# AITRICS/Medical_Tri_Modal_Pilot

Hardware: AMD Instinct MI355X
Metric: tri-modal training samples/s (fwd+bwd+AdamW step, per-GPU batch 64) (higher is better)
Workload: dtype bf16; 1 GPU; BASELINE configs[1]: vslt_img_txt tri_mbt_vsltcls, 6 layers, d_model 256, batch 64/GPU, TIE-len 1000 (N_v=1005), 224x224 CXR, 128-tok text, dropout 0.1, mbt-only-vslt 1, imgtxt-time 1; global_batch=64, parallelism=dp1

## Files before the change

### include/mtmp.h

```cpp
#ifndef MTMP_H
#define MTMP_H
#include <stdint.h>
#ifdef __cplusplus
extern "C" {
#endif

#define MTMP_F32 0
#define MTMP_BF16 1

int mtmp_abi_version(void);
const char* mtmp_last_error(void);

int mtmp_attn_fwd(int dtype, const void* q, const void* k, const void* v, void* o, const void* res, void* o_res,
                  float* lse, const int32_t* kv_len, const float* key_norms, int B, int N, int H, int ld_qkv, int ld_o,
                  float scale, void* stream);
int mtmp_attn_fwd_grouped(int dtype, int n, const void* const* q, const void* const* k, const void* const* v, void* const* o,
                          const void* const* res, void* const* o_res, float* const* lse, const int32_t* const* kv_len,
                          const int32_t* const* row_start, const float* const* key_norms, const int* N, const int* ld_qkv,
                          const int* ld_o, int B, int H, float scale, void* stream);
int mtmp_attn_bwd_grouped(int dtype, int n, const void* const* q, const void* const* k, const void* const* v,
                          const void* const* o, const void* const* d_o, const float* const* lse, const int32_t* const* kv_len,
                          const int32_t* const* row_start, void* const* dq, void* const* dk, void* const* dv,
                          float* const* delta_ws, const int* N, const int* ld_qkv, const int* ld_o, const int* ld_do,
                          const int* ld_dqkv, int B, int H, float scale, void* stream);
int mtmp_attn_cls_fwd(int dtype, const void* q, const void* k, const void* v, int ld_qkv, const void* res, int ld_res, void* o_cls,
                      void* r1_cls, float* lse, const int32_t* kv_len, const int32_t* row_start, int B, int N, int H, int cls_tok,
                      float scale, void* stream);
int mtmp_attn_cls_bwd(int dtype, const void* q, const void* k, const void* v, int ld_qkv, const void* o_cls, const void* d_o,
                      const float* lse, const int32_t* kv_len, const int32_t* row_start, void* dq, void* dk, void* dv, int ld_dqkv,
                      int B, int N, int H, int cls_tok, float scale, void* stream);
long long mtmp_key_norms_floats(long long rows, int H);
int mtmp_key_norms(int dtype, const void* k, float* out, long long rows, int H, int ld, void* stream);

int mtmp_attn_bwd(int dtype, const void* q, const void* k, const void* v, const void* o, const void* d_o,
                  const float* lse, const int32_t* kv_len, void* dq, void* dk, void* dv, float* delta_ws, int B,
                  int N, int H, int ld_qkv, int ld_o, int ld_do, int ld_dqkv, float scale, void* stream);

int mtmp_ln_gemm(int dtype, const void* x, const float* gamma, const float* beta, const void* w, const float* bias,
                 void* y, void* xn, float* stats, int M, int N, int ldx, int ldy, float eps, int relu, float drop_p,
                 unsigned seed, const unsigned* seed_dev, void* stream);

int mtmp_ln_gemm_qkv(int dtype, const void* x, const float* gamma, const float* beta, const void* w, const float* bias,
                     void* y, void* xn, float* stats, float* key_norms, int M, int ldx, float eps, void* stream);

int mtmp_gemm_nt(int dtype, const void* a, const void* w, const float* bias, const void* res, void* y, int M, int N,
                 int K, int lda, int ldy, int ldr, int act, float drop_p, unsigned seed, const unsigned* seed_dev,
                 const void* gate, float gate_scale, const float* row_scale, int rows_per_scale, void* stream);

long long mtmp_sign_bits_bytes(int M, int N);
int mtmp_ln_gemm_signs(int dtype, const void* x, const float* gamma, const float* beta, const void* w, const float* bias,
                       void* y, void* xn, float* stats, int M, int N, int ldx, int ldy, float eps, float drop_p,
                       unsigned seed, const unsigned* seed_dev, void* signs, void* stream);
int mtmp_gemm_nt_signs(int dtype, const void* a, const void* w, void* y, int M, int N, int lda, int ldy,
                       const void* signs, float gate_scale, void* stream);
int mtmp_gemm_nt_signs_drop(int dtype, const void* a, const void* w, void* y, int M, int N, int lda, int ldy,
                            const void* signs, float gate_scale, float drop_p, unsigned seed, const unsigned* seed_dev,
                            void* a_out, void* stream);

long long mtmp_gemm_tn_ws_floats(int M, int N, int K);
int mtmp_gemm_tn(int dtype, const void* dy, const void* x, float* dw, float* db, float* ws, int M, int N, int K,
                 int ldy, int ldx, void* stream);
int mtmp_gemm_tn_live(int dtype, const void* dy, const void* x, float* dw, float* db, float* ws, int M, int N, int K,
                      int ldy, int ldx, const int32_t* rows_live, void* stream);

int mtmp_dropout_bwd(int dtype, const void* g_in, void* g_out, long long n, unsigned seed, const unsigned* seed_dev,
                     float p, void* stream);

int mtmp_ln_bwd_ws_floats(int M);
int mtmp_ln_bwd(int dtype, const void* z, int ldz, const float* stats, const float* gamma, const void* dy,
                const void* d_res, int ldr, void* dz, float* dgamma_dbeta, float* ws, int M, float eps, void* stream);

int mtmp_gemm_lnbwd_ws_floats(int M);
int mtmp_gemm_lnbwd(int dtype, const void* dy, const void* wt, const void* z, int ldz, const float* stats,
                    const float* gamma, const void* d_res, int ldr, void* dz, float* dgamma_dbeta, float* ws, int M,
                    int K, int ldy, float eps, void* stream);

int mtmp_tie_embed_fwd(int dtype, const float* events, const float* params, const float* ftab, void* out, int n,
                       void* stream);
int mtmp_tie_bwd_ws_floats(int n);
int mtmp_tie_embed_bwd(int dtype, const float* events, const float* params, const void* d_out, float* grads,
                       float* ws, int n, void* stream);

int mtmp_time_embed_fwd(int dtype, const float* events, const float* params, const float* ftab, void* out, int n,
// ... 163 lines not shown
```

### medical_tri_modal_pilot_amd/_lib.py

```python
import ctypes
import os
from ctypes import c_char_p, c_float, c_int, c_longlong, c_uint, c_void_p

_HERE = os.path.dirname(os.path.abspath(__file__))
LIB_PATH = os.environ.get("MTMP_LIB", os.path.join(_HERE, "libmtmp_hip.so"))

F32, BF16 = 0, 1

SIGNATURES = {
    "mtmp_abi_version": (c_int, []),
    "mtmp_last_error": (c_char_p, []),
    "mtmp_attn_fwd": (c_int, [c_int] + [c_void_p] * 9 + [c_int] * 5 + [c_float, c_void_p]),
    "mtmp_attn_cls_fwd": (c_int, [c_int] + [c_void_p] * 3 + [c_int, c_void_p, c_int] + [c_void_p] * 5 + [c_int] * 4 + [c_float, c_void_p]),
    "mtmp_attn_cls_bwd": (c_int, [c_int] + [c_void_p] * 3 + [c_int] + [c_void_p] * 8 + [c_int] * 5 + [c_float, c_void_p]),
    "mtmp_attn_fwd_grouped": (c_int, [c_int, c_int] + [c_void_p] * 13 + [c_int, c_int, c_float, c_void_p]),
    "mtmp_attn_bwd_grouped": (c_int, [c_int, c_int] + [c_void_p] * 17 + [c_int, c_int, c_float, c_void_p]),
    "mtmp_key_norms_floats": (c_longlong, [c_longlong, c_int]),
    "mtmp_key_norms": (c_int, [c_int, c_void_p, c_void_p, c_longlong, c_int, c_int, c_void_p]),
    "mtmp_attn_bwd": (c_int, [c_int] + [c_void_p] * 11 + [c_int] * 7 + [c_float, c_void_p]),
    "mtmp_ln_gemm": (c_int, [c_int] + [c_void_p] * 8 + [c_int] * 4 + [c_float, c_int, c_float, c_uint, c_void_p, c_void_p]),
    "mtmp_ln_gemm_qkv": (c_int, [c_int] + [c_void_p] * 9 + [c_int, c_int, c_float, c_void_p]),
    "mtmp_gemm_nt": (c_int, [c_int] + [c_void_p] * 5 + [c_int] * 7 + [c_float, c_uint, c_void_p, c_void_p, c_float, c_void_p, c_int,
                             c_void_p]),
    "mtmp_gemm_nt_live": (c_int, [c_int] + [c_void_p] * 5 + [c_int] * 7 + [c_float, c_uint, c_void_p, c_void_p, c_float, c_void_p, c_int,
                             c_void_p, c_void_p]),
    "mtmp_sign_bits_bytes": (c_longlong, [c_int, c_int]),
    "mtmp_ln_gemm_signs": (c_int, [c_int] + [c_void_p] * 8 + [c_int] * 4 + [c_float, c_float, c_uint, c_void_p, c_void_p, c_void_p]),
    "mtmp_gemm_nt_signs": (c_int, [c_int] + [c_void_p] * 3 + [c_int] * 4 + [c_void_p, c_float, c_void_p]),
    "mtmp_gemm_nt_signs_drop": (c_int, [c_int] + [c_void_p] * 3 + [c_int] * 4 + [c_void_p, c_float, c_float, c_uint, c_void_p,
                                                                                   c_void_p, c_void_p]),
    "mtmp_ln_gemm_qkv_grouped": (c_int, [c_int, c_int] + [c_void_p] * 11 + [c_float, c_void_p, c_void_p]),
    "mtmp_ln_gemm_signs_grouped": (c_int, [c_int, c_int] + [c_void_p] * 10 + [c_int, c_void_p, c_float, c_float, c_void_p, c_void_p,
                                                                                   c_void_p, c_void_p]),
    "mtmp_gemm_nt_grouped": (c_int, [c_int, c_int] + [c_void_p] * 6 + [c_int, c_int] + [c_void_p] * 3 + [c_int, c_float, c_void_p,
                                                                                                       c_void_p, c_void_p, c_void_p]),
    "mtmp_gemm_nt_signs_drop_grouped": (c_int, [c_int, c_int] + [c_void_p] * 4 + [c_int, c_void_p, c_void_p, c_float, c_float,
                                                                                  c_void_p, c_void_p, c_void_p, c_void_p, c_void_p]),
    "mtmp_gemm_lnbwd_grouped": (c_int, [c_int, c_int] + [c_void_p] * 11 + [c_int, c_void_p, c_float, c_void_p, c_void_p]),
    "mtmp_gemm_tn_group_plan": (c_int, [c_int, c_void_p, c_int, c_int, c_void_p]),
    "mtmp_gemm_tn_grouped": (c_int, [c_int, c_int] + [c_void_p] * 4 + [c_int, c_int] + [c_void_p] * 4 + [c_void_p]),
    "mtmp_gemm_tn_slab_rows": (c_int, [c_int] * 4),
    "mtmp_gemm_lnbwd_slab_rows": (c_int, [c_int]),
    "mtmp_reduce_batch": (c_int, [c_void_p] * 6 + [c_int, c_void_p]),
    "mtmp_reduce_scatter": (c_int, [c_void_p] * 5 + [c_int, c_void_p]),
    "mtmp_stream_input_slab_rows": (c_int, [c_int]),
    "mtmp_stream_input_bwd_partials": (c_int, [c_int] + [c_void_p] * 7 + [c_int] * 3 + [c_float, c_uint, c_void_p, c_void_p, c_void_p, c_void_p]),
    "mtmp_stream_input_bwd_grouped": (c_int, [c_int, c_int] + [c_void_p] * 18),
    "mtmp_stream_input_fwd_add": (c_int, [c_int] + [c_void_p] * 8 + [c_int] * 3 + [c_float, c_float, c_uint, c_void_p, c_void_p, c_void_p, c_void_p, c_int, c_void_p]),
    "mtmp_token_sums": (c_int, [c_int, c_int] + [c_void_p] * 5),
    "mtmp_tie_bwd_slab_rows": (c_int, [c_int]),
    "mtmp_tie_time_embed_bwd_partials": (c_int, [c_int, c_void_p, c_int, c_void_p, c_int, c_int] + [c_void_p] * 6),
    "mtmp_publish_scalar": (c_int, [c_void_p, c_void_p, c_void_p]),
    "mtmp_copy_batch": (c_int, [c_void_p] * 4 + [c_int, c_void_p]),
    "mtmp_stream_lengths": (c_int, [c_void_p] * 4 + [c_int] * 3 + [c_void_p]),
    "mtmp_row_starts": (c_int, [c_void_p, c_void_p, c_int, c_int, c_void_p]),
    "mtmp_image_slots": (c_int, [c_void_p, c_int, c_void_p, c_int, c_int, c_void_p]),
    "mtmp_transpose_batch": (c_int, [c_int, c_void_p, c_void_p, c_void_p, c_void_p, c_int, c_void_p]),
    "mtmp_layernorm_rows": (c_int, [c_int] + [c_void_p] * 4 + [c_longlong, c_int, c_float, c_int, c_int, c_int, c_void_p]),
    "mtmp_layernorm_rows_live": (c_int, [c_int] + [c_void_p] * 4 + [c_longlong, c_int, c_float, c_int, c_int, c_int, c_void_p, c_void_p]),
    "mtmp_swin_window_attn": (c_int, [c_int] + [c_void_p] * 3 + [c_int] * 6 + [c_float, c_void_p]),
    "mtmp_swin_window_attn_live": (c_int, [c_int] + [c_void_p] * 3 + [c_int] * 6 + [c_float, c_void_p, c_void_p]),
    "mtmp_layernorm_rows_bwd_slab_rows": (c_int, [c_longlong, c_int]),
    "mtmp_layernorm_rows_bwd": (c_int, [c_int] + [c_void_p] * 5 + [c_longlong, c_int, c_float, c_void_p]),
    "mtmp_gelu_fwd": (c_int, [c_int, c_void_p, c_void_p, c_longlong, c_void_p]),
    "mtmp_gelu_bwd": (c_int, [c_int, c_void_p, c_void_p, c_void_p, c_longlong, c_void_p]),
    "mtmp_swin_window_attn_bwd": (c_int, [c_int] + [c_void_p] * 5 + [c_int] * 6 + [c_float, c_void_p]),
    "mtmp_swin_window_attn_pad": (c_int, [c_int] + [c_void_p] * 4 + [c_int] * 6 + [c_float, c_void_p, c_void_p]),
# ... 67 lines not shown
```

### medical_tri_modal_pilot_amd/ops.py

```python
import contextlib
import ctypes
from typing import Optional

import torch

from . import _lib, tuning
from ._lib import BF16, F32, call

LN_EPS = 1e-6
N_HEAD, D_MODEL, D_HEAD = 4, 256, 64


def _dt(t: torch.Tensor) -> int:
    if t.dtype == torch.float32:
        return F32
    if t.dtype == torch.bfloat16:
        return BF16
    raise TypeError(f"libmtmp_hip kernels take float32 or bfloat16, got {t.dtype}")


def _p(t: Optional[torch.Tensor], byte_offset: int = 0):
    return None if t is None else ctypes.c_void_p(t.data_ptr() + byte_offset)


# ... 1208 lines not shown
        dqkv = attn_bwd(qkv, o, dr1.view(B, N, D), lse, kv_len).view(M, 3 * D)
    else:
        dqkv = attn_bwd_grouped([qkv], [o], [_packed_full(dr1, B, N)], [lse], [kv_len], [pack])[0].view(M, 3 * D)[:live]
    dwqkv, dbqkv = gemm_tn(dqkv, xn1, out=(sink.wqkv, sink.bqkv) if direct else None, defer=red)
    dz, dg1, db1 = gemm_lnbwd(dqkv, wqkvt, z.view(M, D)[:live], st1, g1, d_res2d=dr1, gb_out=sink.gb1 if direct else None, defer=red)
    if late is not None and red:
        late.append((red, sink if direct else None))
    else:
        if red:
            reduce_batch(red)
        if direct:
            sink.flat.mark_ready(sink.idx)
    dz = dz.view(B, N, D) if pack is None else _packed_full(dz, B, N)
    if direct:
        return dz, None
    grads = (dg1, db1, dwqkv[:D], dbqkv[:D], dwqkv[D:2 * D], dbqkv[D:2 * D], dwqkv[2 * D:], dbqkv[2 * D:],
             dg2, db2, dw1, dc1, dw2, dc2)
    return dz, grads


def attn_cls_fwd(qkv, z, kv_len, pack, cls_tok):
    _gpu(qkv, z)
    B, N, _ = qkv.shape
    es = qkv.element_size()
    o = torch.empty(B, D_MODEL, dtype=qkv.dtype, device=qkv.device)
    r1 = torch.empty_like(o)
    lse = torch.empty(B, N_HEAD, dtype=torch.float32, device=qkv.device)
    call("mtmp_attn_cls_fwd", _dt(qkv), _p(qkv), _p(qkv, D_MODEL * es), _p(qkv, 2 * D_MODEL * es), qkv.stride(1), _p(z), z.stride(1),
         _p(o), _p(r1), _p(lse), _p(kv_len), _p(pack), B, N, N_HEAD, int(cls_tok), D_HEAD ** -0.5, _stream())
    return o, r1, lse


def attn_cls_bwd(qkv, o_cls, d_o, lse, kv_len, pack, cls_tok):
    _gpu(qkv, o_cls, d_o)
    B, N, _ = qkv.shape
    es = qkv.element_size()
    dqkv = torch.empty_like(qkv)
    call("mtmp_attn_cls_bwd", _dt(qkv), _p(qkv), _p(qkv, D_MODEL * es), _p(qkv, 2 * D_MODEL * es), qkv.stride(1), _p(o_cls), _p(_c(d_o)),
         _p(lse), _p(kv_len), _p(pack), _p(dqkv), _p(dqkv, D_MODEL * es), _p(dqkv, 2 * D_MODEL * es), dqkv.stride(1), B, N, N_HEAD,
         int(cls_tok), D_HEAD ** -0.5, _stream())
    return dqkv


_cls_rows_cache = {}


def _cls_rows(B, N, cls_tok, dev):
    key = (B, N, cls_tok, dev.type, dev.index)
    if key not in _cls_rows_cache:
        _cls_rows_cache[key] = (torch.arange(B, dtype=torch.int64) * N + cls_tok).to(dev)
    return _cls_rows_cache[key]


def cls_layer_forward(z, kv_len, P, fused, drop_p, seeds, pack, cls_tok):
    B, N, D = z.shape
    g1, b1, g2, b2, c1, c2 = P[0], P[1], P[8], P[9], P[11], P[13]
    wqkv, bqkv, w1c, w2c, w2t, wqkvt, w1t = fused
    z2 = z.view(B * N, D)
    if pack is not None:
        qkv, xn1, st1 = (t[0] for t in ln_gemm_qkv_grouped([z2], [g1], [b1], [wqkv], [bqkv], [pack])[:3])
    else:
        qkv, xn1, st1 = ln_gemm(z2, g1, b1, wqkv, bqkv, 3 * D)
    qkv = qkv.view(B, N, 3 * D)
    o_cls, r1, lse = attn_cls_fwd(qkv, z, kv_len, pack, cls_tok)
    h, xn2, st2, hsign = ln_gemm(r1, g2, b2, w1c, c1, 4 * D, relu=True, drop_p=drop_p, seed=seeds[0], want_signs=True)
    out = gemm_nt(h, w2c, c2, res2d=r1, drop_p=drop_p, seed=seeds[1])
    rows = pack[:B] if pack is not None else _cls_rows(B, N, cls_tok, z.device)
    return out, (z, kv_len, g1, g2, wqkvt, w1t, w2t, xn1, st1, qkv, o_cls, lse, r1, xn2, st2, h, drop_p, seeds, hsign, pack, rows, cls_tok)


def cls_layer_backward(saved, d_cls, sink=None, late=None):
    z, kv_len, g1, g2, wqkvt, w1t, w2t, xn1, st1, qkv, o_cls, lse, r1, xn2, st2, h, p, seeds, hsign, pack, rows, cls_tok = saved
    B, N, D = z.shape
    M = B * N
    d_out = _c(d_cls).to(z.dtype)
    direct = sink is not None and sink.usable()
    red = [] if tuning.DEFER_REDUCTIONS else None
    if hsign is not None and p > 0 and tuning.FOLD_DROPOUT_BWD:
        dh, dy2 = gemm_nt_signs(d_out, w2t, hsign, 1.0 / (1.0 - p), drop_p=p, seed=seeds[1])
    else:
        dy2 = dropout_bwd(d_out, seeds[1], p) if p > 0 else d_out
        dh = gemm_nt_signs(dy2, w2t, hsign, 1.0 / (1.0 - p)) if hsign is not None else gemm_nt(dy2, w2t, gate=h, gate_scale=1.0 / (1.0 - p))
    dw2, dc2 = gemm_tn(dy2, h, out=(sink.w2, sink.c2) if direct else None, defer=red)
    dw1, dc1 = gemm_tn(dh, xn2, out=(sink.w1, sink.c1) if direct else None, defer=red)
    dr1, dg2, db2 = gemm_lnbwd(dh, w1t, r1, st2, g2, d_res2d=d_out, gb_out=sink.gb2 if direct else None, defer=red)
    dqkv = attn_cls_bwd(qkv, o_cls, dr1, lse, kv_len, pack, cls_tok).view(M, 3 * D)
    z2 = z.view(M, D)
    if pack is not None:
        dwqkv, dbqkv = gemm_tn_grouped([dqkv], [xn1], [(sink.wqkv, sink.bqkv) if direct else None], [red], [pack])[0]
        dz, dg1, db1 = gemm_lnbwd_grouped([dqkv], [wqkvt], [z2], [st1], [g1], [None], [sink.gb1 if direct else None], [red], [pack])[0]
    else:
        dwqkv, dbqkv = gemm_tn(dqkv, xn1, out=(sink.wqkv, sink.bqkv) if direct else None, defer=red)
        dz, dg1, db1 = gemm_lnbwd(dqkv, wqkvt, z2, st1, g1, d_res2d=None, gb_out=sink.gb1 if direct else None, defer=red)
    (dz[cls_tok:] if pack is not None else dz).index_add_(0, rows, dr1)
    if late is not None and red:
        late.append((red, sink if direct else None))
    else:
        if red:
            reduce_batch(red)
        if direct:
            sink.flat.mark_ready(sink.idx)
    if direct:
        return dz.view(B, N, D), None
    grads = (dg1, db1, dwqkv[:D], dbqkv[:D], dwqkv[D:2 * D], dbqkv[D:2 * D], dwqkv[2 * D:], dbqkv[2 * D:],
             dg2, db2, dw1, dc1, dw2, dc2)
    return dz.view(B, N, D), grads




def grouped_ok(z) -> bool:
    return tuning.GROUPED_LAUNCHES and z.dtype == torch.bfloat16


def layer_forward_grouped(zs, kv_lens, Ps, fuseds, drop_p, seeds, packs=None, ffn_rows=None):
    n = len(zs)
    B, D = zs[0].shape[0], D_MODEL
    Ns = [z.shape[1] for z in zs]
    packs = [None] * n if packs is None else list(packs)
    z2 = [z.view(B * N, D) for z, N in zip(zs, Ns)]
    qkv, xn1, st1, knorm = ln_gemm_qkv_grouped(z2, [P[0] for P in Ps], [P[1] for P in Ps], [f[0] for f in fuseds], [f[1] for f in fuseds],
                                               packs)
    qkv = [q.view(B, N, 3 * D) for q, N in zip(qkv, Ns)]
    o, r1, lse = attn_fwd_grouped(qkv, kv_lens, list(zs), knorm, packs)
    R = ffn_rows
    if R is not None:
        if any(pk is not None for pk in packs) or any(N < R for N in Ns):
            raise ValueError("ffn_rows: padded streams of at least that many rows")
        r1_2 = [r[:, :R].reshape(B * R, D) for r in r1]
    else:
        r1_2 = [r.view(B * N, D) for r, N in zip(r1, Ns)]
    h, xn2, st2, hsign = ln_gemm_signs_grouped(r1_2, [P[8] for P in Ps], [P[9] for P in Ps], [f[2] for f in fuseds],
                                               [P[11] for P in Ps], 4 * D, drop_p, [sd[0] for sd in seeds], packs)
    out = gemm_nt_grouped(h, [f[3] for f in fuseds], [P[13] for P in Ps], r1_2, drop_p, [sd[1] for sd in seeds], packs)
    if R is not None:
        full = [torch.zeros(B, N, D, dtype=zs[0].dtype, device=zs[0].device) for N in Ns]
        for f_, o_ in zip(full, out):
            f_[:, :R] = o_.view(B, R, D)
        out = full
    saved = [(zs[i], kv_lens[i], Ps[i][0], Ps[i][8], fuseds[i][5], fuseds[i][6], fuseds[i][4], xn1[i], st1[i], qkv[i], o[i], lse[i],
              r1_2[i] if R is not None else r1[i], xn2[i], st2[i], h[i], drop_p, seeds[i], hsign[i], packs[i], R) for i in range(n)]
    return [out[i].view(B, Ns[i], D) for i in range(n)], saved


def layer_backward_grouped(saveds, d_outs, sinks, late):
    n = len(saveds)
    B, D = saveds[0][0].shape[0], D_MODEL
# ... 340 lines not shown
```

### medical_tri_modal_pilot_amd/tuning.py

```python

FOLD_DROPOUT_BWD = True
DEFER_REDUCTIONS = True
LATE_REDUCTIONS = False
GROUPED_LAUNCHES = True
GROUP_MODE = "small"
FFN_ROWS_BEFORE_LAST = True
STREAM_ISSUE_ORDER_FWD = (0, 1, 2)
STREAM_ISSUE_ORDER_BWD = (0, 1, 2)
PREFORK_IMAGE_ENCODER = True
INPUT_NODE_ORDER = "long_last"
FUSED_INPUT_TAIL = True
```

Before: 8278 samples/s.

## Compute CLS-only attention layer with implicit K/V instead of materialized QKV

Adds fused HIP kernels for the CLS-query layer. The forward pass folds the query into W_k so each row only needs its LayerNorm output dotted with a per-head vector, and it accumulates a softmax-weighted sum of the normalized rows before applying W_v once per sample. The full B*N x 3D QKV GEMM, its backward GEMMs and the dense dqkv tensor are no longer materialized for the 1005-token sequence. The cost is custom reduction kernels, a new workspace and partial slabs, and a different summation order that changes numerics.

```diff
diff --git a/include/mtmp.h b/include/mtmp.h
--- a/include/mtmp.h
+++ b/include/mtmp.h
@@ -29,6 +29,16 @@
 int mtmp_attn_cls_bwd(int dtype, const void* q, const void* k, const void* v, int ld_qkv, const void* o_cls, const void* d_o,
                       const float* lse, const int32_t* kv_len, const int32_t* row_start, void* dq, void* dk, void* dv, int ld_dqkv,
                       int B, int N, int H, int cls_tok, float scale, void* stream);
+long long mtmp_cls_kv_fwd_ws_floats(int B, int N);
+long long mtmp_cls_kv_bwd_ws_floats(int B, int N);
+int mtmp_cls_kv_slab_rows(int B, int N);
+int mtmp_cls_kv_fwd(int dtype, const void* z, int ldz, const float* gamma, const float* beta, const void* w, const void* wt,
+                    const float* bias, const int32_t* kv_len, const int32_t* row_start, int B, int N, int cls_tok, float eps,
+                    float scale, float* ws, float* stats, void* r1_cls, void* stream);
+int mtmp_cls_kv_bwd(int dtype, const void* z, int ldz, const float* gamma, const float* beta, const void* w, const void* wt,
+                    const void* d_o, const int32_t* kv_len, const int32_t* row_start, int B, int N, int cls_tok, float eps,
+                    float scale, const float* fwd_ws, const float* stats, float* ws, void* dz, float* slab, float* dw, float* db,
+                    void* stream);
 long long mtmp_key_norms_floats(long long rows, int H);
 int mtmp_key_norms(int dtype, const void* k, float* out, long long rows, int H, int ld, void* stream);
 
diff --git a/medical_tri_modal_pilot_amd/_lib.py b/medical_tri_modal_pilot_amd/_lib.py
--- a/medical_tri_modal_pilot_amd/_lib.py
+++ b/medical_tri_modal_pilot_amd/_lib.py
@@ -13,6 +13,11 @@
     "mtmp_attn_fwd": (c_int, [c_int] + [c_void_p] * 9 + [c_int] * 5 + [c_float, c_void_p]),
     "mtmp_attn_cls_fwd": (c_int, [c_int] + [c_void_p] * 3 + [c_int, c_void_p, c_int] + [c_void_p] * 5 + [c_int] * 4 + [c_float, c_void_p]),
     "mtmp_attn_cls_bwd": (c_int, [c_int] + [c_void_p] * 3 + [c_int] + [c_void_p] * 8 + [c_int] * 5 + [c_float, c_void_p]),
+    "mtmp_cls_kv_fwd_ws_floats": (c_longlong, [c_int, c_int]),
+    "mtmp_cls_kv_bwd_ws_floats": (c_longlong, [c_int, c_int]),
+    "mtmp_cls_kv_slab_rows": (c_int, [c_int, c_int]),
+    "mtmp_cls_kv_fwd": (c_int, [c_int, c_void_p, c_int] + [c_void_p] * 7 + [c_int] * 3 + [c_float, c_float] + [c_void_p] * 4),
+    "mtmp_cls_kv_bwd": (c_int, [c_int, c_void_p, c_int] + [c_void_p] * 7 + [c_int] * 3 + [c_float, c_float] + [c_void_p] * 8),
     "mtmp_attn_fwd_grouped": (c_int, [c_int, c_int] + [c_void_p] * 13 + [c_int, c_int, c_float, c_void_p]),
     "mtmp_attn_bwd_grouped": (c_int, [c_int, c_int] + [c_void_p] * 17 + [c_int, c_int, c_float, c_void_p]),
     "mtmp_key_norms_floats": (c_longlong, [c_longlong, c_int]),
diff --git a/medical_tri_modal_pilot_amd/csrc/cls_layer.hip b/medical_tri_modal_pilot_amd/csrc/cls_layer.hip
--- /dev/null
+++ b/medical_tri_modal_pilot_amd/csrc/cls_layer.hip
@@ -0,0 +1,479 @@
+#include "common.hip.h"
+
+namespace {
+constexpr int D = 256, H = 4, DH = 64, CH = 128;
+constexpr int RPW = 4;
+constexpr float LOG2E = 1.4426950408889634f, LN2 = 0.6931471805599453f;
+constexpr int CTX_A = 0, CTX_U = 1024, CTX_Q = 2048, CTX_X = 2304, CTX_LSE = 2560, CTX = 2568;
+constexpr int PART_M = 1024, PART_L = 1028, PART = 1032;
+constexpr int BCTX_C = 0, BCTX_T = 1024, BCTX_DQ = 2048, BCTX_CU = 2304, BCTX = 2312;
+
+template <typename T> struct ClsKvArgs {
+    const T* z; int ldz;
+    const float* gamma; const float* beta;
+    const T* w; const T* wt;
+    const float* bias;
+    const int* kv_len; const int* row_start;
+    int B, N, cls_tok, nchunk;
+    float eps, scale;
+    float* ctx; float* part; float* stats;
+    T* r1;
+    const T* d_o;
+    float* bctx; float* tpart;
+    T* dz; float* slab;
+    float* dw; float* db;
+};
+
+struct Rows { size_t row0; int kvl, nrows; bool uniform; };
+template <typename T> MTMP_DEV Rows sample_rows(const ClsKvArgs<T>& p, int b) {
+    const int kv_raw = p.kv_len ? p.kv_len[b] : p.N;
+    Rows r;
+    r.row0 = p.row_start ? (size_t)p.row_start[b] : (size_t)b * p.N;
+    if (p.row_start && kv_raw <= p.cls_tok) { r.kvl = 0; r.nrows = 0; r.uniform = false; return r; }
+    r.uniform = kv_raw <= 0;
+    r.kvl = r.uniform ? p.N : min(kv_raw, p.N);
+    r.nrows = p.row_start ? r.kvl : p.N;
+    return r;
+}
+
+MTMP_DEV float block_sum(float v, float* red) {
+    v = wave_sum(v);
+    __syncthreads();
+    if ((threadIdx.x & 63) == 0) red[threadIdx.x >> 6] = v;
+    __syncthreads();
+    return (red[0] + red[1]) + (red[2] + red[3]);
+}
+
+template <typename T> MTMP_DEV void matvec_t(const T* wt, int ldw, const float* v, int vstride, float* part, int lane, int wave) {
+    const float* vv = v + (lane >> 4) * vstride;
+    float acc[4] = {0.f, 0.f, 0.f, 0.f};
+#pragma unroll 8
+    for (int i = 0; i < 64; ++i) {
+        const int k = 64 * wave + i;
+        const f32x4 wv = load4<T>(wt + (size_t)k * ldw + 4 * lane);
+        const float x = vv[k];
+#pragma unroll
+        for (int j = 0; j < 4; ++j) acc[j] = fmaf(x, wv[j], acc[j]);
+    }
+    *reinterpret_cast<f32x4*>(part + wave * D + 4 * lane) = f32x4{acc[0], acc[1], acc[2], acc[3]};
+}
+MTMP_DEV float part_sum(const float* part, int i) { return (part[i] + part[D + i]) + (part[2 * D + i] + part[3 * D + i]); }
+
+template <typename T> MTMP_DEV void headvec(const T* w, const float* u, float (&acc)[4], int lane, int wave) {
+#pragma unroll
+    for (int j = 0; j < 4; ++j) acc[j] = 0.f;
+#pragma unroll 8
+    for (int d = 0; d < DH; ++d) {
+        const int n = DH * wave + d;
+        const f32x4 wv = load4<T>(w + (size_t)n * D + 4 * lane);
+        const float x = u[n];
+#pragma unroll
+        for (int j = 0; j < 4; ++j) acc[j] = fmaf(x, wv[j], acc[j]);
+    }
+}
+
+MTMP_DEV void ln_row_block(float v, float eps, float* red, float& xh, float& rs, float& sigma) {
+    const float mean = block_sum(v, red) * (1.0f / D);
+    const float d = v - mean;
+    sigma = sqrtf(block_sum(d * d, red) * (1.0f / (D - 1)));
+    rs = 1.0f / (sigma + eps);
+    xh = d * rs;
+}
+
+template <typename T> __global__ __launch_bounds__(256) void cls_kv_query_kernel(ClsKvArgs<T> p) {
+    __shared__ __attribute__((aligned(16))) float sv[D], part[4 * D];
+    __shared__ float red[4];
+    const int b = blockIdx.x, tid = threadIdx.x, lane = tid & 63, wave = tid >> 6;
+    const Rows r = sample_rows(p, b);
+    float* ctx = p.ctx + (size_t)b * CTX;
+    if (r.kvl == 0) {
+        for (int i = tid; i < CTX; i += 256) ctx[i] = 0.f;
+        return;
+    }
+    float xh, rs, sigma;
+    ln_row_block(to_f32(p.z[(r.row0 + p.cls_tok) * p.ldz + tid]), p.eps, red, xh, rs, sigma);
+    const float x = fmaf(p.gamma[tid], xh, p.beta[tid]);
+    ctx[CTX_X + tid] = x;
+    sv[tid] = x;
+    __syncthreads();
+    matvec_t<T>(p.wt, 3 * D, sv, 0, part, lane, wave);
+    __syncthreads();
+    const float q = part_sum(part, tid) + p.bias[tid];
+    ctx[CTX_Q + tid] = q;
+    sv[tid] = q;
+    __syncthreads();
+    float a[4];
+    headvec<T>(p.w + (size_t)D * D, sv, a, lane, wave);
+    const float c2 = r.uniform ? 0.f : p.scale * LOG2E;
+    *reinterpret_cast<f32x4*>(ctx + CTX_A + wave * D + 4 * lane) = f32x4{a[0] * c2, a[1] * c2, a[2] * c2, a[3] * c2};
+}
+
+template <typename T, int NV> __global__ __launch_bounds__(256) void cls_kv_rows_fwd_kernel(ClsKvArgs<T> p) {
+    __shared__ __attribute__((aligned(16))) float su[4 * NV * D];
+    __shared__ float sm[4 * NV], sl[4 * NV];
+    const int ci = blockIdx.x, b = blockIdx.y, tid = threadIdx.x, lane = tid & 63, wave = tid >> 6;
+    const Rows r = sample_rows(p, b);
+    const f32x4 gm = ld4f(p.gamma + 4 * lane), be = ld4f(p.beta + 4 * lane);
+    f32x4 a[NV];
+#pragma unroll
+    for (int h = 0; h < NV; ++h) a[h] = ld4f(p.ctx + (size_t)b * CTX + CTX_A + h * D + 4 * lane);
+    float m[NV], l[NV], acc[NV][4];
+#pragma unroll
+    for (int h = 0; h < NV; ++h) { m[h] = -INFINITY; l[h] = 0.f; acc[h][0] = acc[h][1] = acc[h][2] = acc[h][3] = 0.f; }
+    const int rb = ci * CH + wave * (CH / 4);
+    for (int t = 0; t < CH / 4 / RPW; ++t) {
+        const int r0 = rb + RPW * t;
+        if (r0 >= r.kvl) break;
+        f32x4 zv[RPW];
+#pragma unroll
+        for (int k = 0; k < RPW; ++k) zv[k] = load4<T>(p.z + (r.row0 + min(r0 + k, r.kvl - 1)) * p.ldz + 4 * lane);
+        float x[RPW][4], s[RPW][NV];
+#pragma unroll
+        for (int k = 0; k < RPW; ++k) {
+            const bool valid = r0 + k < r.kvl;
+            const float mean = wave_sum((zv[k][0] + zv[k][1]) + (zv[k][2] + zv[k][3])) * (1.0f / D);
+            float d[4], s2 = 0.f;
+#pragma unroll
+            for (int i = 0; i < 4; ++i) { d[i] = zv[k][i] - mean; s2 = fmaf(d[i], d[i], s2); }
+            const float rs = 1.0f / (sqrtf(wave_sum(s2) * (1.0f / (D - 1))) + p.eps);
+#pragma unroll
+            for (int i = 0; i < 4; ++i) x[k][i] = fmaf(gm[i], d[i] * rs, be[i]);
+            if (valid && lane == 0) {
+                float* st = p.stats + 2 * (r.row0 + r0 + k);
+                st[0] = mean;
+                st[1] = rs;
+            }
+#pragma unroll
+            for (int h = 0; h < NV; ++h) {
+                float dot = 0.f;
+#pragma unroll
+                for (int i = 0; i < 4; ++i) dot = fmaf(a[h][i], x[k][i], dot);
+                dot = wave_sum(dot);
+                s[k][h] = valid ? dot : -INFINITY;
+            }
+        }
+#pragma unroll
+        for (int h = 0; h < NV; ++h) {
+            float mn = m[h];
+#pragma unroll
+            for (int k = 0; k < RPW; ++k) mn = fmaxf(mn, s[k][h]);
+            const float f = fast_exp2(m[h] - mn);
+            m[h] = mn;
+            l[h] *= f;
+#pragma unroll
+            for (int i = 0; i < 4; ++i) acc[h][i] *= f;
+#pragma unroll
+            for (int k = 0; k < RPW; ++k) {
+                const float e = fast_exp2(s[k][h] - mn);
+                l[h] += e;
+#pragma unroll
+                for (int i = 0; i < 4; ++i) acc[h][i] = fmaf(e, x[k][i], acc[h][i]);
+            }
+        }
+    }
+#pragma unroll
+    for (int h = 0; h < NV; ++h) {
+        *reinterpret_cast<f32x4*>(su + (wave * NV + h) * D + 4 * lane) = f32x4{acc[h][0], acc[h][1], acc[h][2], acc[h][3]};
+        if (lane == 0) { sm[wave * NV + h] = m[h]; sl[wave * NV + h] = l[h]; }
+    }
+    __syncthreads();
+    float* out = p.part + ((size_t)b * p.nchunk + ci) * (NV * D + 2 * NV);
+#pragma unroll
+    for (int h = 0; h < NV; ++h) {
+        const float mx = fmaxf(fmaxf(sm[h], sm[NV + h]), fmaxf(sm[2 * NV + h], sm[3 * NV + h]));
+        float u = 0.f, ls = 0.f;
+        if (mx > -INFINITY) {
+#pragma unroll
+            for (int w = 0; w < 4; ++w) {
+                const float f = fast_exp2(sm[w * NV + h] - mx);
+                u = fmaf(f, su[(w * NV + h) * D + tid], u);
+                ls = fmaf(f, sl[w * NV + h], ls);
+            }
+        }
+        out[h * D + tid] = u;
+        if (tid == 0) { out[NV * D + h] = mx; out[NV * D + NV + h] = ls; }
+    }
+}
+
+template <typename T> __global__ __launch_bounds__(256) void cls_kv_combine_kernel(ClsKvArgs<T> p) {
+    __shared__ __attribute__((aligned(16))) float su[H * D], part[4 * D];
+    const int b = blockIdx.x, tid = threadIdx.x, lane = tid & 63, wave = tid >> 6;
+    const Rows r = sample_rows(p, b);
+    if (r.kvl == 0) {
+        p.r1[(size_t)b * D + tid] = from_f32<T>(0.f);
+        return;
+    }
+    float* ctx = p.ctx + (size_t)b * CTX;
+    const float* pp = p.part + (size_t)b * p.nchunk * PART;
+#pragma unroll
+    for (int h = 0; h < H; ++h) {
+        float mx = -INFINITY;
+        for (int c = 0; c < p.nchunk; ++c) mx = fmaxf(mx, pp[c * PART + PART_M + h]);
+        float u = 0.f, ls = 0.f;
+        for (int c = 0; c < p.nchunk; ++c) {
+            const float f = fast_exp2(pp[c * PART + PART_M + h] - mx);
+            u = fmaf(f, pp[c * PART + h * D + tid], u);
+            ls = fmaf(f, pp[c * PART + PART_L + h], ls);
+        }
+        u /= ls;
+        ctx[CTX_U + h * D + tid] = u;
+        su[h * D + tid] = u;
+        if (tid == 0) ctx[CTX_LSE + h] = mx + log2f(ls);
+    }
+    __syncthreads();
+    matvec_t<T>(p.wt + 2 * D, 3 * D, su, D, part, lane, wave);
+    __syncthreads();
+    const float o = round_as<T>(part_sum(part, tid) + p.bias[2 * D + tid]);
+    p.r1[(size_t)b * D + tid] = from_f32<T>(o + to_f32(p.z[(r.row0 + p.cls_tok) * p.ldz + tid]));
+}
+
+template <typename T> __global__ __launch_bounds__(256) void cls_kv_bwd_query_kernel(ClsKvArgs<T> p) {
+    __shared__ float sg[D];
+    const int b = blockIdx.x, tid = threadIdx.x, lane = tid & 63, wave = tid >> 6;
+    sg[tid] = to_f32(p.d_o[(size_t)b * D + tid]);
+    __syncthreads();
+    float c[4];
+    headvec<T>(p.w + (size_t)2 * D * D, sg, c, lane, wave);
+    const f32x4 u = ld4f(p.ctx + (size_t)b * CTX + CTX_U + wave * D + 4 * lane);
+    float* bc = p.bctx + (size_t)b * BCTX;
+    *reinterpret_cast<f32x4*>(bc + BCTX_C + wave * D + 4 * lane) = f32x4{c[0], c[1], c[2], c[3]};
+    const float cu = wave_sum(fmaf(c[0], u[0], c[1] * u[1]) + fmaf(c[2], u[2], c[3] * u[3]));
+    if (lane == 0) bc[BCTX_CU + wave] = cu;
+}
+
+template <typename T, int NV> __global__ __launch_bounds__(256) void cls_kv_rows_bwd_kernel(ClsKvArgs<T> p) {
+    __shared__ __attribute__((aligned(16))) float lds[4 * NV * D];
+    const int ci = blockIdx.x, b = blockIdx.y, tid = threadIdx.x, lane = tid & 63, wave = tid >> 6;
+    const Rows r = sample_rows(p, b);
+    const f32x4 gm = ld4f(p.gamma + 4 * lane), be = ld4f(p.beta + 4 * lane);
+    const float* ctx = p.ctx + (size_t)b * CTX;
+    const float* bc = p.bctx + (size_t)b * BCTX;
+    f32x4 a[NV], c[NV];
+    float lse[NV], cu[NV];
+#pragma unroll
+    for (int h = 0; h < NV; ++h) {
+        a[h] = ld4f(ctx + CTX_A + h * D + 4 * lane);
+        c[h] = ld4f(bc + BCTX_C + h * D + 4 * lane);
+        lse[h] = ctx[CTX_LSE + h];
+        cu[h] = bc[BCTX_CU + h];
+    }
+    float tacc[NV][4], gb[2][4] = {{0.f, 0.f, 0.f, 0.f}, {0.f, 0.f, 0.f, 0.f}};
+#pragma unroll
+    for (int h = 0; h < NV; ++h) tacc[h][0] = tacc[h][1] = tacc[h][2] = tacc[h][3] = 0.f;
+    const float dsw = r.uniform ? 0.f : 1.f;
+    const int rb = ci * CH + wave * (CH / 4);
+    for (int t = 0; t < CH / 4 / RPW; ++t) {
+        const int r0 = rb + RPW * t;
+        if (r0 >= r.nrows) break;
+        if (r0 >= r.kvl) {
+            for (int k = 0; k < RPW && r0 + k < r.nrows; ++k) store4<T>(p.dz + (r.row0 + r0 + k) * D + 4 * lane, 0.f, 0.f, 0.f, 0.f);
+            continue;
+        }
+        f32x4 zv[RPW];
+        float mu[RPW], rs[RPW];
+#pragma unroll
+        for (int k = 0; k < RPW; ++k) {
+            const size_t row = r.row0 + min(r0 + k, r.kvl - 1);
+            zv[k] = load4<T>(p.z + row * p.ldz + 4 * lane);
+            mu[k] = p.stats[2 * row];
+            rs[k] = p.stats[2 * row + 1];
+        }
+#pragma unroll
+        for (int k = 0; k < RPW; ++k) {
+            const int rr = r0 + k;
+            const float live = rr < r.kvl ? 1.f : 0.f;
+            float xh[4], x[4], dx[4] = {0.f, 0.f, 0.f, 0.f};
+#pragma unroll
+            for (int i = 0; i < 4; ++i) { xh[i] = (zv[k][i] - mu[k]) * rs[k]; x[i] = fmaf(gm[i], xh[i], be[i]); }
+#pragma unroll
+            for (int h = 0; h < NV; ++h) {
+                float s = 0.f, cx = 0.f;
+#pragma unroll
+                for (int i = 0; i < 4; ++i) { s = fmaf(a[h][i], x[i], s); cx = fmaf(c[h][i], x[i], cx); }
+                wave_sum2(s, cx);
+                const float pj = fast_exp2(s - lse[h]);
+                const float ds = dsw * pj * (cx - cu[h]);
+                const float dsa = ds * LN2;
+#pragma unroll
+                for (int i = 0; i < 4; ++i) {
+                    dx[i] = fmaf(dsa, a[h][i], fmaf(pj, c[h][i], dx[i]));
+                    tacc[h][i] = fmaf(live * ds, x[i], tacc[h][i]);
+                }
+            }
+            const float own = (rr < r.kvl && rr != p.cls_tok) ? 1.f : 0.f;
+            float g[4], sg = 0.f, sgx = 0.f;
+#pragma unroll
+            for (int i = 0; i < 4; ++i) {
+                g[i] = dx[i] * gm[i];
+                sg += g[i];
+                sgx = fmaf(g[i], xh[i], sgx);
+                gb[0][i] = fmaf(own * dx[i], xh[i], gb[0][i]);
+                gb[1][i] = fmaf(own, dx[i], gb[1][i]);
+            }
+            wave_sum2(sg, sgx);
+            const float mg = sg * (1.0f / D);
+            const float kx = sgx / ((float)(D - 1) * (1.0f / rs[k] - p.eps));
+            if (rr < r.kvl)
+                store4<T>(p.dz + (r.row0 + rr) * D + 4 * lane, (g[0] - mg) * rs[k] - xh[0] * kx, (g[1] - mg) * rs[k] - xh[1] * kx,
+                          (g[2] - mg) * rs[k] - xh[2] * kx, (g[3] - mg) * rs[k] - xh[3] * kx);
+            else if (rr < r.nrows)
+                store4<T>(p.dz + (r.row0 + rr) * D + 4 * lane, 0.f, 0.f, 0.f, 0.f);
+        }
+    }
+    const size_t wg = (size_t)b * p.nchunk + ci;
+    flush_partials<NV>(tacc, p.tpart + wg * NV * D, lds, lane, wave);
+    __syncthreads();
+    flush_partials<2>(gb, p.slab + wg * 2 * D, lds, lane, wave);
+}
+
+template <typename T> __global__ __launch_bounds__(256) void cls_kv_bwd_finish_kernel(ClsKvArgs<T> p) {
+    __shared__ __attribute__((aligned(16))) float sv[H * D], part[4 * D], sx[D];
+    __shared__ float red[4], sp[H], sds[H];
+    const int b = blockIdx.x, tid = threadIdx.x, lane = tid & 63, wave = tid >> 6;
+    const Rows r = sample_rows(p, b);
+    float* bc = p.bctx + (size_t)b * BCTX;
+    float* slab = p.slab + ((size_t)p.B * p.nchunk + b) * 2 * D;
+    if (r.kvl == 0) {
+        for (int i = tid; i < BCTX; i += 256) bc[i] = 0.f;
+        slab[tid] = 0.f;
+        slab[D + tid] = 0.f;
+        return;
+    }
+    const float* ctx = p.ctx + (size_t)b * CTX;
+#pragma unroll
+    for (int h = 0; h < H; ++h) {
+        const float* tp = p.tpart + (size_t)b * p.nchunk * H * D + h * D + tid;
+        float t = 0.f;
+        for (int c = 0; c < p.nchunk; ++c) t += tp[(size_t)c * H * D];
+        bc[BCTX_T + h * D + tid] = t;
+        sv[h * D + tid] = t;
+    }
+    __syncthreads();
+    matvec_t<T>(p.wt + D, 3 * D, sv, D, part, lane, wave);
+    __syncthreads();
+    const float dq = p.scale * part_sum(part, tid);
+    bc[BCTX_DQ + tid] = dq;
+    sx[tid] = dq;
+    __syncthreads();
+    float e4[4];
+    headvec<T>(p.w, sx, e4, lane, wave);
+    __syncthreads();
+    *reinterpret_cast<f32x4*>(part + wave * D + 4 * lane) = f32x4{e4[0], e4[1], e4[2], e4[3]};
+    const size_t rowc = r.row0 + p.cls_tok;
+    float xh, rs, sigma;
+    ln_row_block(to_f32(p.z[rowc * p.ldz + tid]), p.eps, red, xh, rs, sigma);
+    const float x = fmaf(p.gamma[tid], xh, p.beta[tid]);
+    sx[tid] = x;
+    __syncthreads();
+    {
+        const f32x4 a = ld4f(ctx + CTX_A + wave * D + 4 * lane), c = ld4f(bc + BCTX_C + wave * D + 4 * lane);
+        const f32x4 xv = ld4f(sx + 4 * lane);
+        float s = fmaf(a[0], xv[0], a[1] * xv[1]) + fmaf(a[2], xv[2], a[3] * xv[3]);
+        float cx = fmaf(c[0], xv[0], c[1] * xv[1]) + fmaf(c[2], xv[2], c[3] * xv[3]);
+        wave_sum2(s, cx);
+        const float pj = p.cls_tok < r.kvl ? fast_exp2(s - ctx[CTX_LSE + wave]) : 0.f;
+        if (lane == 0) { sp[wave] = pj; sds[wave] = r.uniform ? 0.f : pj * (cx - bc[BCTX_CU + wave]); }
+    }
+    __syncthreads();
+    float dx = part_sum(part, tid);
+#pragma unroll
+    for (int h = 0; h < H; ++h) dx = fmaf(sds[h] * LN2, ctx[CTX_A + h * D + tid], fmaf(sp[h], bc[BCTX_C + h * D + tid], dx));
+    const float g = dx * p.gamma[tid];
+    const float mg = block_sum(g, red) * (1.0f / D);
+    const float kx = block_sum(g * xh, red) / ((float)(D - 1) * sigma);
+    p.dz[rowc * D + tid] = from_f32<T>((g - mg) * rs - xh * kx + to_f32(p.d_o[(size_t)b * D + tid]));
+    slab[tid] = dx * xh;
+    slab[D + tid] = dx;
+}
+
+template <typename T> __global__ __launch_bounds__(256) void cls_kv_wgrad_kernel(ClsKvArgs<T> p) {
+    const int tid = threadIdx.x, n0 = 4 * blockIdx.x, sec = n0 / D, h = (n0 % D) / DH;
+    float acc[4] = {0.f, 0.f, 0.f, 0.f}, bs[4] = {0.f, 0.f, 0.f, 0.f};
+    for (int b = 0; b < p.B; ++b) {
+        const float* ctx = p.ctx + (size_t)b * CTX;
+        const float* bc = p.bctx + (size_t)b * BCTX;
+        const int kv_raw = p.kv_len ? p.kv_len[b] : p.N;
+        if (p.row_start && kv_raw <= p.cls_tok) continue;
+        const float right = sec == 0 ? ctx[CTX_X + tid] : sec == 1 ? bc[BCTX_T + h * D + tid] : ctx[CTX_U + h * D + tid];
+#pragma unroll
+        for (int j = 0; j < 4; ++j) {
+            const int n = n0 % D + j;
+            const float left = sec == 0 ? bc[BCTX_DQ + n] : sec == 1 ? p.scale * ctx[CTX_Q + n] : to_f32(p.d_o[(size_t)b * D + n]);
+            acc[j] = fmaf(left, right, acc[j]);
+            bs[j] += left;
+        }
+    }
+#pragma unroll
+    for (int j = 0; j < 4; ++j) {
+        p.dw[(size_t)(n0 + j) * D + tid] = acc[j];
+        if (tid == 0) p.db[n0 + j] = sec == 1 ? 0.f : bs[j];
+    }
+}
+
+bool cls_kv_ok(int B, int N, int cls_tok, int ldz) {
+    return B > 0 && N > 0 && N <= 8192 && cls_tok >= 0 && cls_tok < N && ldz >= D && ldz % 4 == 0;
+}
+int chunks(int N) { return (N + CH - 1) / CH; }
+
+template <typename T> void launch_fwd(const ClsKvArgs<T>& a, hipStream_t st) {
+    hipLaunchKernelGGL(cls_kv_query_kernel<T>, dim3(a.B), dim3(256), 0, st, a);
+    hipLaunchKernelGGL((cls_kv_rows_fwd_kernel<T, H>), dim3(a.nchunk, a.B), dim3(256), 0, st, a);
+    hipLaunchKernelGGL(cls_kv_combine_kernel<T>, dim3(a.B), dim3(256), 0, st, a);
+}
+template <typename T> void launch_bwd(const ClsKvArgs<T>& a, hipStream_t st) {
+    hipLaunchKernelGGL(cls_kv_bwd_query_kernel<T>, dim3(a.B), dim3(256), 0, st, a);
+    hipLaunchKernelGGL((cls_kv_rows_bwd_kernel<T, H>), dim3(a.nchunk, a.B), dim3(256), 0, st, a);
+    hipLaunchKernelGGL(cls_kv_bwd_finish_kernel<T>, dim3(a.B), dim3(256), 0, st, a);
+    hipLaunchKernelGGL(cls_kv_wgrad_kernel<T>, dim3(3 * D / 4), dim3(256), 0, st, a);
+}
+}
+
+extern "C" long long mtmp_cls_kv_fwd_ws_floats(int B, int N) { return (long long)B * CTX + (long long)B * chunks(N) * PART; }
+extern "C" long long mtmp_cls_kv_bwd_ws_floats(int B, int N) { return (long long)B * BCTX + (long long)B * chunks(N) * H * D; }
+extern "C" int mtmp_cls_kv_slab_rows(int B, int N) { return B * chunks(N) + B; }
+
+extern "C" int mtmp_cls_kv_fwd(int dtype, const void* z, int ldz, const float* gamma, const float* beta, const void* w, const void* wt,
+                               const float* bias, const int32_t* kv_len, const int32_t* row_start, int B, int N, int cls_tok, float eps,
+                               float scale, float* ws, float* stats, void* r1_cls, void* stream) {
+    MTMP_CHECK_ARG(z && gamma && beta && w && wt && bias && ws && stats && r1_cls, "mtmp_cls_kv_fwd: null pointer");
+    MTMP_CHECK_ARG(cls_kv_ok(B, N, cls_tok, ldz) && (!row_start || kv_len), "mtmp_cls_kv_fwd: bad argument (B=%d N=%d cls=%d ld=%d)", B, N,
+                   cls_tok, ldz);
+    hipStream_t st = (hipStream_t)stream;
+    if (dtype == 0) {
+        ClsKvArgs<float> a{(const float*)z, ldz, gamma, beta, (const float*)w, (const float*)wt, bias, kv_len, row_start, B, N, cls_tok,
+                           chunks(N), eps, scale, ws, ws + (size_t)B * CTX, stats, (float*)r1_cls, nullptr, nullptr, nullptr, nullptr,
+                           nullptr, nullptr, nullptr};
+        launch_fwd(a, st);
+    } else if (dtype == 1) {
+        ClsKvArgs<bf16> a{(const bf16*)z, ldz, gamma, beta, (const bf16*)w, (const bf16*)wt, bias, kv_len, row_start, B, N, cls_tok,
+                          chunks(N), eps, scale, ws, ws + (size_t)B * CTX, stats, (bf16*)r1_cls, nullptr, nullptr, nullptr, nullptr,
+                          nullptr, nullptr, nullptr};
+        launch_fwd(a, st);
+    } else { mtmp_set_error("mtmp_cls_kv_fwd: unknown dtype %d", dtype); return MTMP_ERR_ARG; }
+    MTMP_CHECK_LAUNCH("mtmp_cls_kv_fwd");
+    return MTMP_OK;
+}
+
+extern "C" int mtmp_cls_kv_bwd(int dtype, const void* z, int ldz, const float* gamma, const float* beta, const void* w, const void* wt,
+                               const void* d_o, const int32_t* kv_len, const int32_t* row_start, int B, int N, int cls_tok, float eps,
+                               float scale, const float* fwd_ws, const float* stats, float* ws, void* dz, float* slab, float* dw,
+                               float* db, void* stream) {
+    MTMP_CHECK_ARG(z && gamma && beta && w && wt && d_o && fwd_ws && stats && ws && dz && slab && dw && db, "mtmp_cls_kv_bwd: null pointer");
+    MTMP_CHECK_ARG(cls_kv_ok(B, N, cls_tok, ldz) && (!row_start || kv_len), "mtmp_cls_kv_bwd: bad argument (B=%d N=%d cls=%d ld=%d)", B, N,
+                   cls_tok, ldz);
+    hipStream_t st = (hipStream_t)stream;
+    float* fws = const_cast<float*>(fwd_ws);
+    if (dtype == 0) {
+        ClsKvArgs<float> a{(const float*)z, ldz, gamma, beta, (const float*)w, (const float*)wt, nullptr, kv_len, row_start, B, N,
+                           cls_tok, chunks(N), eps, scale, fws, nullptr, const_cast<float*>(stats), nullptr, (const float*)d_o, ws,
+                           ws + (size_t)B * BCTX, (float*)dz, slab, dw, db};
+        launch_bwd(a, st);
+    } else if (dtype == 1) {
+        ClsKvArgs<bf16> a{(const bf16*)z, ldz, gamma, beta, (const bf16*)w, (const bf16*)wt, nullptr, kv_len, row_start, B, N, cls_tok,
+                          chunks(N), eps, scale, fws, nullptr, const_cast<float*>(stats), nullptr, (const bf16*)d_o, ws,
+                          ws + (size_t)B * BCTX, (bf16*)dz, slab, dw, db};
+        launch_bwd(a, st);
+    } else { mtmp_set_error("mtmp_cls_kv_bwd: unknown dtype %d", dtype); return MTMP_ERR_ARG; }
+    MTMP_CHECK_LAUNCH("mtmp_cls_kv_bwd");
+    return MTMP_OK;
+}
diff --git a/medical_tri_modal_pilot_amd/ops.py b/medical_tri_modal_pilot_amd/ops.py
--- a/medical_tri_modal_pilot_amd/ops.py
+++ b/medical_tri_modal_pilot_amd/ops.py
@@ -1284,25 +1284,65 @@
     return _cls_rows_cache[key]
 
 
+def cls_kv_fwd(z, gamma, beta, wqkv, wqkvt, bqkv, kv_len, pack, cls_tok):
+    _gpu(z, wqkv, wqkvt)
+    B, N, _ = z.shape
+    ws = torch.empty(_lib.lib().mtmp_cls_kv_fwd_ws_floats(B, N), dtype=torch.float32, device=z.device)
+    stats = torch.empty(B * N, 2, dtype=torch.float32, device=z.device)
+    r1 = torch.empty(B, D_MODEL, dtype=z.dtype, device=z.device)
+    call("mtmp_cls_kv_fwd", _dt(z), _p(z), z.stride(1), _p(gamma), _p(beta), _p(wqkv), _p(wqkvt), _p(bqkv), _p(kv_len), _p(pack), B, N,
+         int(cls_tok), LN_EPS, D_HEAD ** -0.5, _p(ws), _p(stats), _p(r1), _stream())
+    return r1, (ws, stats)
+
+
+def cls_kv_bwd(z, gamma, beta, wqkv, wqkvt, d_o, kv_len, pack, cls_tok, state, out=None, gb_out=None, defer=None, dz=None):
+    _gpu(z, d_o)
+    B, N, _ = z.shape
+    dev = z.device
+    ws_f, stats = state
+    if dz is None:
+        dz = torch.empty(B * N, D_MODEL, dtype=z.dtype, device=dev)
+    dw, db = out if out is not None else (torch.empty(3 * D_MODEL, D_MODEL, dtype=torch.float32, device=dev),
+                                          torch.empty(3 * D_MODEL, dtype=torch.float32, device=dev))
+    gb = gb_out if gb_out is not None else torch.empty(2 * D_MODEL, dtype=torch.float32, device=dev)
+    rows = _lib.lib().mtmp_cls_kv_slab_rows(B, N)
+    slab = torch.empty(rows, 2 * D_MODEL, dtype=torch.float32, device=dev)
+    ws = torch.empty(_lib.lib().mtmp_cls_kv_bwd_ws_floats(B, N), dtype=torch.float32, device=dev)
+    call("mtmp_cls_kv_bwd", _dt(z), _p(z), z.stride(1), _p(gamma), _p(beta), _p(wqkv), _p(wqkvt), _p(_c(d_o)), _p(kv_len), _p(pack), B, N,
+         int(cls_tok), LN_EPS, D_HEAD ** -0.5, _p(ws_f), _p(stats), _p(ws), _p(dz), _p(slab), _p(dw), _p(db), _stream())
+    entry = [(slab, rows, 2 * D_MODEL, gb, 2 * D_MODEL, None)]
+    if defer is not None:
+        defer.extend(entry)
+    else:
+        reduce_batch(entry)
+    return dz, gb[:D_MODEL], gb[D_MODEL:], dw, db
+
+
 def cls_layer_forward(z, kv_len, P, fused, drop_p, seeds, pack, cls_tok):
     B, N, D = z.shape
     g1, b1, g2, b2, c1, c2 = P[0], P[1], P[8], P[9], P[11], P[13]
     wqkv, bqkv, w1c, w2c, w2t, wqkvt, w1t = fused
     z2 = z.view(B * N, D)
-    if pack is not None:
-        qkv, xn1, st1 = (t[0] for t in ln_gemm_qkv_grouped([z2], [g1], [b1], [wqkv], [bqkv], [pack])[:3])
+    xn1 = st1 = qkv = o_cls = lse = kvs = None
+    if tuning.CLS_IMPLICIT_KV and z.dtype == torch.bfloat16:
+        r1, state = cls_kv_fwd(z, g1, b1, wqkv, wqkvt, bqkv, kv_len, pack, cls_tok)
+        kvs = (b1, wqkv) + state
     else:
-        qkv, xn1, st1 = ln_gemm(z2, g1, b1, wqkv, bqkv, 3 * D)
-    qkv = qkv.view(B, N, 3 * D)
-    o_cls, r1, lse = attn_cls_fwd(qkv, z, kv_len, pack, cls_tok)
+        if pack is not None:
+            qkv, xn1, st1 = (t[0] for t in ln_gemm_qkv_grouped([z2], [g1], [b1], [wqkv], [bqkv], [pack])[:3])
+        else:
+            qkv, xn1, st1 = ln_gemm(z2, g1, b1, wqkv, bqkv, 3 * D)
+        qkv = qkv.view(B, N, 3 * D)
+        o_cls, r1, lse = attn_cls_fwd(qkv, z, kv_len, pack, cls_tok)
     h, xn2, st2, hsign = ln_gemm(r1, g2, b2, w1c, c1, 4 * D, relu=True, drop_p=drop_p, seed=seeds[0], want_signs=True)
     out = gemm_nt(h, w2c, c2, res2d=r1, drop_p=drop_p, seed=seeds[1])
     rows = pack[:B] if pack is not None else _cls_rows(B, N, cls_tok, z.device)
-    return out, (z, kv_len, g1, g2, wqkvt, w1t, w2t, xn1, st1, qkv, o_cls, lse, r1, xn2, st2, h, drop_p, seeds, hsign, pack, rows, cls_tok)
+    return out, (z, kv_len, g1, g2, wqkvt, w1t, w2t, xn1, st1, qkv, o_cls, lse, r1, xn2, st2, h, drop_p, seeds, hsign, pack, rows, cls_tok,
+                 kvs)
 
 
 def cls_layer_backward(saved, d_cls, sink=None, late=None):
-    z, kv_len, g1, g2, wqkvt, w1t, w2t, xn1, st1, qkv, o_cls, lse, r1, xn2, st2, h, p, seeds, hsign, pack, rows, cls_tok = saved
+    z, kv_len, g1, g2, wqkvt, w1t, w2t, xn1, st1, qkv, o_cls, lse, r1, xn2, st2, h, p, seeds, hsign, pack, rows, cls_tok, kvs = saved
     B, N, D = z.shape
     M = B * N
     d_out = _c(d_cls).to(z.dtype)
@@ -1316,15 +1356,20 @@
     dw2, dc2 = gemm_tn(dy2, h, out=(sink.w2, sink.c2) if direct else None, defer=red)
     dw1, dc1 = gemm_tn(dh, xn2, out=(sink.w1, sink.c1) if direct else None, defer=red)
     dr1, dg2, db2 = gemm_lnbwd(dh, w1t, r1, st2, g2, d_res2d=d_out, gb_out=sink.gb2 if direct else None, defer=red)
-    dqkv = attn_cls_bwd(qkv, o_cls, dr1, lse, kv_len, pack, cls_tok).view(M, 3 * D)
-    z2 = z.view(M, D)
-    if pack is not None:
-        dwqkv, dbqkv = gemm_tn_grouped([dqkv], [xn1], [(sink.wqkv, sink.bqkv) if direct else None], [red], [pack])[0]
-        dz, dg1, db1 = gemm_lnbwd_grouped([dqkv], [wqkvt], [z2], [st1], [g1], [None], [sink.gb1 if direct else None], [red], [pack])[0]
+    if kvs is not None:
+        dz, dg1, db1, dwqkv, dbqkv = cls_kv_bwd(z, g1, kvs[0], kvs[1], wqkvt, dr1, kv_len, pack, cls_tok, kvs[2:],
+                                                out=(sink.wqkv, sink.bqkv) if direct else None,
+                                                gb_out=sink.gb1 if direct else None, defer=red)
     else:
-        dwqkv, dbqkv = gemm_tn(dqkv, xn1, out=(sink.wqkv, sink.bqkv) if direct else None, defer=red)
-        dz, dg1, db1 = gemm_lnbwd(dqkv, wqkvt, z2, st1, g1, d_res2d=None, gb_out=sink.gb1 if direct else None, defer=red)
-    (dz[cls_tok:] if pack is not None else dz).index_add_(0, rows, dr1)
+        dqkv = attn_cls_bwd(qkv, o_cls, dr1, lse, kv_len, pack, cls_tok).view(M, 3 * D)
+        z2 = z.view(M, D)
+        if pack is not None:
+            dwqkv, dbqkv = gemm_tn_grouped([dqkv], [xn1], [(sink.wqkv, sink.bqkv) if direct else None], [red], [pack])[0]
+            dz, dg1, db1 = gemm_lnbwd_grouped([dqkv], [wqkvt], [z2], [st1], [g1], [None], [sink.gb1 if direct else None], [red], [pack])[0]
+        else:
+            dwqkv, dbqkv = gemm_tn(dqkv, xn1, out=(sink.wqkv, sink.bqkv) if direct else None, defer=red)
+            dz, dg1, db1 = gemm_lnbwd(dqkv, wqkvt, z2, st1, g1, d_res2d=None, gb_out=sink.gb1 if direct else None, defer=red)
+        (dz[cls_tok:] if pack is not None else dz).index_add_(0, rows, dr1)
     if late is not None and red:
         late.append((red, sink if direct else None))
     else:
diff --git a/medical_tri_modal_pilot_amd/tuning.py b/medical_tri_modal_pilot_amd/tuning.py
--- a/medical_tri_modal_pilot_amd/tuning.py
+++ b/medical_tri_modal_pilot_amd/tuning.py
@@ -5,6 +5,7 @@
 GROUPED_LAUNCHES = True
 GROUP_MODE = "small"
 FFN_ROWS_BEFORE_LAST = True
+CLS_IMPLICIT_KV = True
 STREAM_ISSUE_ORDER_FWD = (0, 1, 2)
 STREAM_ISSUE_ORDER_BWD = (0, 1, 2)
 PREFORK_IMAGE_ENCODER = True
```

Measured after the change: 8348 samples/s (median of 6 runs). Within noise of the previous version (+0.8%).
